# abdur75648/AI-Camera

Hardware: AMD Instinct MI355X
Metric: end-to-end frames/sec @1280x720, 30 persons/frame (higher is better)
Workload: dtype f16

## Files before the change

### ai-camera_amd/csrc/kernels_conv_block.hip

```cpp
#include "conv_common.hpp"

namespace aic {

struct BlockArgs {
    const void* x; void* y;
    const void* w1; const float* b1;
    const void* w2; const float* b2;
    const void* zero;
    int x_cs, x_coff, y_cs, y_coff, H, n_img, ipb;
    const int* n_dev;
};

__global__ __launch_bounds__(512) void conv3x3_c64_block_kernel(const BlockArgs a) {
    constexpr int PW = 34, ROWB = PW * 128, IN_ROWS = 20, MID_ROWS = 16;
    constexpr int MID_OFF = IN_ROWS * ROWB, DUMMY_OFF = MID_OFF + MID_ROWS * ROWB, BIAS_OFF = DUMMY_OFF + 1024;
    extern __shared__ __attribute__((aligned(16))) char smem[];

    const int t = threadIdx.x, lane = t & 63, wv = __builtin_amdgcn_readfirstlane(t >> 6), r = lane & 15, q = lane >> 4;
    const int grp = wv >> 2, cx = wv & 1, ch = (wv >> 1) & 1;
    const half_t* __restrict__ xg = reinterpret_cast<const half_t*>(a.x);
    const half_t* zero = reinterpret_cast<const half_t*>(a.zero);
    const half_t* __restrict__ wg = reinterpret_cast<const half_t*>(grp ? a.w2 : a.w1);
    const float* bg = grp ? a.b2 : a.b1;

    half8 wreg[18][2];
#pragma unroll
    for (int j = 0; j < 2; ++j) {
        const half_t* wr = wg + (size_t)(32 * ch + perm_row<2>(j, r)) * 576 + 8 * q;
#pragma unroll
        for (int s2 = 0; s2 < 18; ++s2) wreg[s2][j] = *reinterpret_cast<const half8*>(wr + 32 * s2);
    }
#pragma unroll
    for (int s2 = 0; s2 < 18; ++s2) asm volatile("" :: "v"(wreg[s2][0]), "v"(wreg[s2][1]));
    float* bias_l = reinterpret_cast<float*>(smem + BIAS_OFF) + ((grp * 2 + ch) * 4 + q) * 8;
    if (cx == 0 && r == 0) {
#pragma unroll
        for (int j = 0; j < 2; ++j)
#pragma unroll
            for (int e = 0; e < 4; ++e) bias_l[4 * j + e] = bg[32 * ch + perm_ch<2>(j, q, e)];
    }
    for (int o = t * 16; o < MID_ROWS * ROWB; o += 512 * 16) *reinterpret_cast<uint4*>(smem + MID_OFF + o) = make_uint4(0u, 0u, 0u, 0u);

    const int gpi = a.H / 4 + 1;
    const int n_live = a.n_dev ? min(a.n_img, a.n_dev[0]) : a.n_img;
    const int ipb = a.n_dev ? (n_live + (int)gridDim.x - 1) / (int)gridDim.x : a.ipb;
    const int img0 = blockIdx.x * ipb;
    const int n_loc = max(0, min(ipb, n_live - img0));
    const int S_tot = gpi * n_loc;

    int doff[3];
#pragma unroll
    for (int p = 0; p < 3; ++p) {
        const int sl = (p * 8 + wv) * 64 + lane;
        const int rr = sl / 272, rem = sl - rr * 272;
        const int px = rem >> 3, c = (rem & 7) ^ (px & 7);
        doff[p] = (p * 8 + wv < 17 && (unsigned)(px - 1) < 32u) ? (rr * 32 + (px - 1)) * a.x_cs + a.x_coff + c * 8 : -1;
    }
    auto issue = [&](int g) {
        int gs = g % 5; if (gs < 0) gs += 5;
        const int jl = g >= 0 ? g / gpi : 0, gy = g - jl * gpi;
        const bool real = g >= 0 && jl < n_loc && gy < gpi - 1;
        const half_t* gbase = xg + ((size_t)(img0 + jl) * a.H + gy * 4) * 32 * a.x_cs;
#pragma unroll
        for (int p = 0; p < 3; ++p) {
            const int j = p * 8 + wv;
            const half_t* src = (real && doff[p] >= 0) ? gbase + doff[p] : zero;
            asm volatile("" : "+v"(src));
            char* dst = j < 17 ? smem + gs * 4 * ROWB + j * 1024 : smem + DUMMY_OFF;
            __builtin_amdgcn_global_load_lds((gptr_t)src, (lptr_t)dst, 16, 0, 0);
        }
    };

    int xk[3];
#pragma unroll
    for (int kw = 0; kw < 3; ++kw) {
        const int px = cx * 16 + r + kw;
        xk[kw] = (px * 8 + (q ^ (px & 7))) * 16;
    }
    const int px1 = cx * 16 + r + 1;
    const int mid_w = (px1 * 8 + ((4 * ch + q) ^ (px1 & 7))) * 16;

    half_t* yg = reinterpret_cast<half_t*>(a.y);
    const unsigned yl0 = (unsigned)((((cx * 16 + r) * a.y_cs) + a.y_coff + 32 * ch + 8 * q) * 2);
    const unsigned rl0 = (unsigned)((((cx * 16 + r) * a.x_cs) + a.x_coff + 32 * ch + 8 * q) * 2);
    const unsigned ystep = (unsigned)(32 * a.y_cs * 2), rstep = (unsigned)(32 * a.x_cs * 2);

    floatx4 acc[4][2];
    half8 rv[4];
    half8 xf[6];
    int rowb[6];
    auto xread = [&xf, &xk, &rowb](auto g, auto ir) {
        constexpr int gg = decltype(g)::value, ii = decltype(ir)::value, kw = gg >> 1;
        const int ad = ((gg & 1) ? (xk[kw] ^ 64) : xk[kw]) + rowb[ii];
        asm volatile("ds_read_b128 %0, %1" : "=v"(xf[ii]) : "v"(ad));
    };
    auto xwait = [&xf](auto n, auto ir) {
        asm volatile("s_waitcnt lgkmcnt(%1)" : "+v"(xf[decltype(ir)::value]) : "n"(decltype(n)::value));
    };
    auto kfirst = [&]() {
        static_for<6>([&](auto ir) { xread(std::integral_constant<int, 0>{}, ir); });
#pragma unroll
        for (int i = 0; i < 4; ++i)
#pragma unroll
            for (int j = 0; j < 2; ++j) acc[i][j] = *reinterpret_cast<const floatx4*>(bias_l + 4 * j);
    };
    auto kpart = [&](auto part) {
        static_for<3>([&](auto gi) {
            constexpr int g = 3 * decltype(part)::value + decltype(gi)::value, kw = g >> 1, cc = g & 1;
            static_for<6>([&](auto ir_c) {
                constexpr int ir = decltype(ir_c)::value;
                xwait(std::integral_constant<int, (g == 5 ? 5 - ir : 5)>{}, ir_c);
#pragma unroll
                for (int kh = 0; kh < 3; ++kh) {
                    const int i = ir - kh;
                    if (i < 0 || i > 3) continue;
#pragma unroll
                    for (int j = 0; j < 2; ++j)
                        acc[i][j] = __builtin_amdgcn_mfma_f32_16x16x32_f16(wreg[(kh * 3 + kw) * 2 + cc][j], xf[ir], acc[i][j], 0, 0, 0);
                }
                if constexpr (g + 1 < 6) xread(std::integral_constant<int, g + 1>{}, ir_c);
                __builtin_amdgcn_sched_barrier(0);
            });
        });
    };
    using P0 = std::integral_constant<int, 0>;
    using P1 = std::integral_constant<int, 1>;

    auto rows1 = [&](int s) {
#pragma unroll
        for (int ir = 0; ir < 6; ++ir) {
            const int v = 4 * s - 1 + ir;
            int gsl = (v >> 2) % 5; if (gsl < 0) gsl += 5;
            rowb[ir] = (gsl * 4 + (v & 3)) * ROWB;
        }
    };
    auto store_mid = [&](int s) {
#pragma unroll
        for (int i = 0; i < 4; ++i) {
            float v[8];
#pragma unroll
            for (int e = 0; e < 8; ++e) v[e] = act_fast<2>(acc[i][e >> 2][e & 3]);
            const half8 o = {(half_t)v[0], (half_t)v[1], (half_t)v[2], (half_t)v[3], (half_t)v[4], (half_t)v[5], (half_t)v[6], (half_t)v[7]};
            const int ad = MID_OFF + ((4 * s + i) & 15) * ROWB + mid_w;
            asm volatile("ds_write_b128 %0, %1" :: "v"(ad), "v"(o) : "memory");
        }
    };
    auto zero_mid = [&](int s) {
        const half8 o = {0, 0, 0, 0, 0, 0, 0, 0};
#pragma unroll
        for (int i = 0; i < 4; ++i) {
            const int ad = MID_OFF + ((4 * s + i) & 15) * ROWB + mid_w;
            asm volatile("ds_write_b128 %0, %1" :: "v"(ad), "v"(o) : "memory");
        }
    };
    auto load_res = [&](size_t pix0) {
        const char* rb = reinterpret_cast<const char*>(xg) + pix0 * a.x_cs * 2;
        unsigned rl = rl0;
        asm volatile("" : "+v"(rl));
#pragma unroll
        for (int i = 0; i < 4; ++i)
            asm volatile("global_load_dwordx4 %0, %1, %2" : "=v"(rv[i]) : "v"(rl + i * rstep), "s"(rb) : "memory");
    };
    auto rows2 = [&](int tt) {
#pragma unroll
        for (int ir = 0; ir < 6; ++ir) rowb[ir] = MID_OFF + ((4 * tt - 1 + ir) & 15) * ROWB;
    };
    auto store_out = [&](size_t pix0) {
        asm volatile("s_waitcnt vmcnt(3)" : "+v"(rv[0]), "+v"(rv[1]), "+v"(rv[2]), "+v"(rv[3]) :: "memory");
        char* yb = reinterpret_cast<char*>(yg) + pix0 * a.y_cs * 2;
        unsigned yl = yl0;
        asm volatile("" : "+v"(yl));
#pragma unroll
        for (int i = 0; i < 4; ++i) {
            float v[8];
#pragma unroll
            for (int e = 0; e < 8; ++e) v[e] = act_fast<2>(acc[i][e >> 2][e & 3] + (float)rv[i][e]);
            const half8 o = {(half_t)v[0], (half_t)v[1], (half_t)v[2], (half_t)v[3], (half_t)v[4], (half_t)v[5], (half_t)v[6], (half_t)v[7]};
            *reinterpret_cast<half8*>(yb + (size_t)(yl + i * ystep)) = o;
        }
    };

    issue(-1); issue(0); issue(1); issue(2);
    asm volatile("s_waitcnt lgkmcnt(0)" ::: "memory");
    if (grp == 0) {
        for (int s = 0; s < S_tot + 2; ++s) {
            wait_vmcnt<3>();
            __builtin_amdgcn_s_barrier();
            issue(s + 3);
            const bool live = s < S_tot, act1 = live && s % gpi < gpi - 1;
            if (act1) {
                rows1(s);
                kfirst();
                kpart(P0{});
            }
            __builtin_amdgcn_s_barrier();
            if (live) {
                if (act1) {
                    kpart(P1{});
                    store_mid(s);
                } else zero_mid(s);
                asm volatile("s_waitcnt lgkmcnt(0)" ::: "memory");
            }
        }
        __builtin_amdgcn_s_barrier();
    } else {
        wait_vmcnt<3>();
        __builtin_amdgcn_s_barrier();
        bool prev = false;
        for (int s = 0; s < S_tot + 2; ++s) {
            __builtin_amdgcn_s_barrier();
            const int tt = s - 2;
            const bool act2 = tt >= 0 && tt < S_tot && (tt % gpi) < gpi - 1;
            const int jl = act2 ? tt / gpi : 0, gy = act2 ? tt % gpi : 0;
            const size_t pix0 = ((size_t)(img0 + jl) * a.H + gy * 4) * 32;
            if (act2) load_res(pix0);
            issue(s + 3);
            if (act2) {
                rows2(tt);
                kfirst();
                kpart(P0{});
            }
            if (act2 && prev) wait_vmcnt<11>();
            else if (act2 || prev) wait_vmcnt<7>();
            else wait_vmcnt<3>();
            __builtin_amdgcn_s_barrier();
            if (act2) {
                kpart(P1{});
                store_out(pix0);
            }
            prev = act2;
        }
    }
    wait_vmcnt<0>();
}

void launch_c64_block(const ConvArgs& c1, const ConvArgs& c2, int ipb, hipStream_t s) {
    BlockArgs a{};
    a.x = c1.x, a.y = c2.y, a.w1 = c1.w, a.b1 = c1.bias, a.w2 = c2.w, a.b2 = c2.bias, a.zero = c1.zero;
    a.x_cs = c1.x_cs, a.x_coff = c1.x_coff, a.y_cs = c2.y_cs, a.y_coff = c2.y_coff, a.H = c1.H;
    a.n_img = c1.M / (c1.H * c1.W);
    a.n_dev = c1.n_dev;
    a.ipb = ipb;
    constexpr size_t lds = (size_t)(20 + 16) * 34 * 128 + 1024 + 512;
    set_lds_limit(conv3x3_c64_block_kernel, lds);
    hipLaunchKernelGGL(conv3x3_c64_block_kernel, dim3((a.n_img + a.ipb - 1) / a.ipb), dim3(512), lds, s, a);
    KCHECK();
}

}
```

Before: 13120.

## Interleave epilogue stores with final MFMA group and strength-reduce block conv indexing

The fused two-conv block kernel now emits the mid-row LDS writes and output global stores inside the last MFMA group instead of after it, so the epilogue overlaps with matrix work. Bias initialisation is done through two LDS reads feeding the first MFMA accumulator. Per-step divisions and modulos for slot and row addressing are replaced with incrementally updated counters and pointers. Wave priority is raised around the second half. Optional compile-time timestamp instrumentation is added but disabled by default. The waitcnt arithmetic gets more intricate, which raises the risk of ordering mistakes.

```diff
diff --git a/ai-camera_amd/csrc/kernels_conv_block.hip b/ai-camera_amd/csrc/kernels_conv_block.hip
--- a/ai-camera_amd/csrc/kernels_conv_block.hip
+++ b/ai-camera_amd/csrc/kernels_conv_block.hip
@@ -1,6 +1,25 @@
 #include "conv_common.hpp"
 
 namespace aic {
+
+#ifdef AICAM_BLOCK_STAMPS
+constexpr int STAMP_BLOCKS = 1536, STAMP_WORDS = 16;
+__device__ unsigned long long aic_block_stamp_buf[STAMP_BLOCKS * 8 * STAMP_WORDS];
+struct BlockStamps { unsigned long long t[6], sum[6], steps, last, t_begin, rt_begin; bool have; };
+#define BLK_STAMP(k) do { __builtin_amdgcn_sched_barrier(0); asm volatile("s_memtime %0\n\ts_waitcnt lgkmcnt(0)" : "=s"(st.t[k]) :: "memory"); __builtin_amdgcn_sched_barrier(0); } while (0)
+#define BLK_TOP() do { if (st.have) st.sum[5] += st.t[0] - st.last; st.have = false; } while (0)
+#define BLK_STEP() do { for (int k_ = 0; k_ < 5; ++k_) st.sum[k_] += st.t[k_ + 1] - st.t[k_]; ++st.steps; st.last = st.t[5]; st.have = true; } while (0)
+#define BLK_STAMPS_BEGIN() BlockStamps st{}; asm volatile("s_memtime %0\n\ts_memrealtime %1\n\ts_waitcnt lgkmcnt(0)" : "=s"(st.t_begin), "=s"(st.rt_begin) :: "memory")
+#define BLK_STAMPS_OUT() do { unsigned long long te_, re_; asm volatile("s_memtime %0\n\ts_memrealtime %1\n\ts_waitcnt lgkmcnt(0)" : "=s"(te_), "=s"(re_) :: "memory"); \
+        if (lane == 0 && blockIdx.x < STAMP_BLOCKS) { unsigned long long* o_ = aic_block_stamp_buf + ((size_t)blockIdx.x * 8 + wv) * STAMP_WORDS; \
+            for (int k_ = 0; k_ < 6; ++k_) o_[k_] = st.sum[k_]; o_[6] = st.steps; o_[7] = te_ - st.t_begin; o_[8] = re_ - st.rt_begin; } } while (0)
+#else
+#define BLK_STAMP(k) do {} while (0)
+#define BLK_TOP() do {} while (0)
+#define BLK_STEP() do {} while (0)
+#define BLK_STAMPS_BEGIN() do {} while (0)
+#define BLK_STAMPS_OUT() do {} while (0)
+#endif
 
 struct BlockArgs {
     const void* x; void* y;
@@ -39,6 +58,7 @@
 #pragma unroll
             for (int e = 0; e < 4; ++e) bias_l[4 * j + e] = bg[32 * ch + perm_ch<2>(j, q, e)];
     }
+    const int bias_ad = BIAS_OFF + ((grp * 2 + ch) * 4 + q) * 32;
     for (int o = t * 16; o < MID_ROWS * ROWB; o += 512 * 16) *reinterpret_cast<uint4*>(smem + MID_OFF + o) = make_uint4(0u, 0u, 0u, 0u);
 
     const int gpi = a.H / 4 + 1;
@@ -56,11 +76,7 @@
         const int px = rem >> 3, c = (rem & 7) ^ (px & 7);
         doff[p] = (p * 8 + wv < 17 && (unsigned)(px - 1) < 32u) ? (rr * 32 + (px - 1)) * a.x_cs + a.x_coff + c * 8 : -1;
     }
-    auto issue = [&](int g) {
-        int gs = g % 5; if (gs < 0) gs += 5;
-        const int jl = g >= 0 ? g / gpi : 0, gy = g - jl * gpi;
-        const bool real = g >= 0 && jl < n_loc && gy < gpi - 1;
-        const half_t* gbase = xg + ((size_t)(img0 + jl) * a.H + gy * 4) * 32 * a.x_cs;
+    auto issue_at = [&](int gs, bool real, const half_t* gbase) {
 #pragma unroll
         for (int p = 0; p < 3; ++p) {
             const int j = p * 8 + wv;
@@ -70,6 +86,16 @@
             __builtin_amdgcn_global_load_lds((gptr_t)src, (lptr_t)dst, 16, 0, 0);
         }
     };
+    int i_gs = 4, i_jl = 0, i_gy = -1;
+    const half_t* i_ptr = xg + (size_t)img0 * a.H * 32 * a.x_cs;
+    const size_t i_step = (size_t)4 * 32 * a.x_cs;
+    auto issue_next = [&]() {
+        const bool real = i_gy >= 0 && i_jl < n_loc && i_gy < gpi - 1;
+        issue_at(i_gs, real, i_ptr);
+        if (i_gy >= 0 && i_gy < gpi - 1) i_ptr += i_step;
+        i_gs = i_gs == 4 ? 0 : i_gs + 1;
+        if (++i_gy == gpi) i_gy = 0, ++i_jl;
+    };
 
     int xk[3];
 #pragma unroll
@@ -89,6 +115,7 @@
     half8 rv[4];
     half8 xf[6];
     int rowb[6];
+    BLK_STAMPS_BEGIN();
     auto xread = [&xf, &xk, &rowb](auto g, auto ir) {
         constexpr int gg = decltype(g)::value, ii = decltype(ir)::value, kw = gg >> 1;
         const int ad = ((gg & 1) ? (xk[kw] ^ 64) : xk[kw]) + rowb[ii];
@@ -98,52 +125,55 @@
         asm volatile("s_waitcnt lgkmcnt(%1)" : "+v"(xf[decltype(ir)::value]) : "n"(decltype(n)::value));
     };
     auto kfirst = [&]() {
+        asm volatile("ds_read_b128 %0, %1" : "=v"(acc[3][0]) : "v"(bias_ad));
+        asm volatile("ds_read_b128 %0, %1 offset:16" : "=v"(acc[3][1]) : "v"(bias_ad));
         static_for<6>([&](auto ir) { xread(std::integral_constant<int, 0>{}, ir); });
-#pragma unroll
-        for (int i = 0; i < 4; ++i)
-#pragma unroll
-            for (int j = 0; j < 2; ++j) acc[i][j] = *reinterpret_cast<const floatx4*>(bias_l + 4 * j);
-    };
-    auto kpart = [&](auto part) {
+    };
+    auto kpart = [&](auto part, auto lds_writes, auto&& tail) {
         static_for<3>([&](auto gi) {
             constexpr int g = 3 * decltype(part)::value + decltype(gi)::value, kw = g >> 1, cc = g & 1;
             static_for<6>([&](auto ir_c) {
                 constexpr int ir = decltype(ir_c)::value;
-                xwait(std::integral_constant<int, (g == 5 ? 5 - ir : 5)>{}, ir_c);
+                constexpr int wr = g == 5 && decltype(lds_writes)::value && ir > 2 ? ir - 2 : 0;
+                xwait(std::integral_constant<int, (g == 5 ? 5 - ir + wr : 5)>{}, ir_c);
+                if constexpr (g == 0 && ir == 0) asm volatile("" : "+v"(acc[3][0]), "+v"(acc[3][1]));
 #pragma unroll
                 for (int kh = 0; kh < 3; ++kh) {
                     const int i = ir - kh;
                     if (i < 0 || i > 3) continue;
 #pragma unroll
                     for (int j = 0; j < 2; ++j)
-                        acc[i][j] = __builtin_amdgcn_mfma_f32_16x16x32_f16(wreg[(kh * 3 + kw) * 2 + cc][j], xf[ir], acc[i][j], 0, 0, 0);
+                        acc[i][j] = __builtin_amdgcn_mfma_f32_16x16x32_f16(wreg[(kh * 3 + kw) * 2 + cc][j], xf[ir], (g == 0 && kh == 0) ? acc[3][j] : acc[i][j], 0, 0, 0);
                 }
                 if constexpr (g + 1 < 6) xread(std::integral_constant<int, g + 1>{}, ir_c);
                 __builtin_amdgcn_sched_barrier(0);
+                if constexpr (g == 5 && ir == 5) BLK_STAMP(4);
+                if constexpr (g == 5 && ir >= 2) {
+                    tail(std::integral_constant<int, ir - 2>{});
+                    __builtin_amdgcn_sched_barrier(0);
+                }
             });
         });
     };
     using P0 = std::integral_constant<int, 0>;
     using P1 = std::integral_constant<int, 1>;
-
-    auto rows1 = [&](int s) {
-#pragma unroll
-        for (int ir = 0; ir < 6; ++ir) {
-            const int v = 4 * s - 1 + ir;
-            int gsl = (v >> 2) % 5; if (gsl < 0) gsl += 5;
-            rowb[ir] = (gsl * 4 + (v & 3)) * ROWB;
-        }
-    };
-    auto store_mid = [&](int s) {
-#pragma unroll
-        for (int i = 0; i < 4; ++i) {
-            float v[8];
-#pragma unroll
-            for (int e = 0; e < 8; ++e) v[e] = act_fast<2>(acc[i][e >> 2][e & 3]);
-            const half8 o = {(half_t)v[0], (half_t)v[1], (half_t)v[2], (half_t)v[3], (half_t)v[4], (half_t)v[5], (half_t)v[6], (half_t)v[7]};
-            const int ad = MID_OFF + ((4 * s + i) & 15) * ROWB + mid_w;
-            asm volatile("ds_write_b128 %0, %1" :: "v"(ad), "v"(o) : "memory");
-        }
+    auto no_tail = [](auto) {};
+
+    auto rows1 = [&](int s5) {
+        const int up = s5 == 0 ? 4 : s5 - 1, dn = s5 == 4 ? 0 : s5 + 1;
+        rowb[0] = (up * 4 + 3) * ROWB;
+#pragma unroll
+        for (int ir = 1; ir < 5; ++ir) rowb[ir] = (s5 * 4 + ir - 1) * ROWB;
+        rowb[5] = dn * 4 * ROWB;
+    };
+    auto mid_row = [&](int s, auto ic) {
+        constexpr int i = decltype(ic)::value;
+        float v[8];
+#pragma unroll
+        for (int e = 0; e < 8; ++e) v[e] = act_fast<2>(acc[i][e >> 2][e & 3]);
+        const half8 o = {(half_t)v[0], (half_t)v[1], (half_t)v[2], (half_t)v[3], (half_t)v[4], (half_t)v[5], (half_t)v[6], (half_t)v[7]};
+        const int ad = MID_OFF + ((4 * s + i) & 15) * ROWB + mid_w;
+        asm volatile("ds_write_b128 %0, %1" :: "v"(ad), "v"(o) : "memory");
     };
     auto zero_mid = [&](int s) {
         const half8 o = {0, 0, 0, 0, 0, 0, 0, 0};
@@ -153,8 +183,7 @@
             asm volatile("ds_write_b128 %0, %1" :: "v"(ad), "v"(o) : "memory");
         }
     };
-    auto load_res = [&](size_t pix0) {
-        const char* rb = reinterpret_cast<const char*>(xg) + pix0 * a.x_cs * 2;
+    auto load_res = [&](const char* rb) {
         unsigned rl = rl0;
         asm volatile("" : "+v"(rl));
 #pragma unroll
@@ -165,73 +194,92 @@
 #pragma unroll
         for (int ir = 0; ir < 6; ++ir) rowb[ir] = MID_OFF + ((4 * tt - 1 + ir) & 15) * ROWB;
     };
-    auto store_out = [&](size_t pix0) {
-        asm volatile("s_waitcnt vmcnt(3)" : "+v"(rv[0]), "+v"(rv[1]), "+v"(rv[2]), "+v"(rv[3]) :: "memory");
-        char* yb = reinterpret_cast<char*>(yg) + pix0 * a.y_cs * 2;
+    auto out_row = [&](char* yb, auto ic) {
+        constexpr int i = decltype(ic)::value;
+        if constexpr (i == 0) asm volatile("s_waitcnt vmcnt(3)" : "+v"(rv[0]), "+v"(rv[1]), "+v"(rv[2]), "+v"(rv[3]) :: "memory");
         unsigned yl = yl0;
         asm volatile("" : "+v"(yl));
-#pragma unroll
-        for (int i = 0; i < 4; ++i) {
-            float v[8];
-#pragma unroll
-            for (int e = 0; e < 8; ++e) v[e] = act_fast<2>(acc[i][e >> 2][e & 3] + (float)rv[i][e]);
-            const half8 o = {(half_t)v[0], (half_t)v[1], (half_t)v[2], (half_t)v[3], (half_t)v[4], (half_t)v[5], (half_t)v[6], (half_t)v[7]};
-            *reinterpret_cast<half8*>(yb + (size_t)(yl + i * ystep)) = o;
-        }
-    };
-
-    issue(-1); issue(0); issue(1); issue(2);
+        float v[8];
+#pragma unroll
+        for (int e = 0; e < 8; ++e) v[e] = act_fast<2>(acc[i][e >> 2][e & 3] + (float)rv[i][e]);
+        const half8 o = {(half_t)v[0], (half_t)v[1], (half_t)v[2], (half_t)v[3], (half_t)v[4], (half_t)v[5], (half_t)v[6], (half_t)v[7]};
+        *reinterpret_cast<half8*>(yb + (size_t)(yl + i * ystep)) = o;
+    };
+
+    issue_next(); issue_next(); issue_next(); issue_next();
     asm volatile("s_waitcnt lgkmcnt(0)" ::: "memory");
     if (grp == 0) {
+        int sy = 0, s5 = 0;
         for (int s = 0; s < S_tot + 2; ++s) {
             wait_vmcnt<3>();
             __builtin_amdgcn_s_barrier();
-            issue(s + 3);
-            const bool live = s < S_tot, act1 = live && s % gpi < gpi - 1;
+            BLK_STAMP(0);
+            BLK_TOP();
+            issue_next();
+            const bool live = s < S_tot, act1 = live && sy < gpi - 1;
             if (act1) {
-                rows1(s);
+                BLK_STAMP(1);
+                rows1(s5);
                 kfirst();
-                kpart(P0{});
+                kpart(P0{}, std::true_type{}, no_tail);
+                BLK_STAMP(2);
             }
             __builtin_amdgcn_s_barrier();
             if (live) {
                 if (act1) {
-                    kpart(P1{});
-                    store_mid(s);
+                    BLK_STAMP(3);
+                    __builtin_amdgcn_s_setprio(1);
+                    kpart(P1{}, std::true_type{}, [&](auto i) { mid_row(s, i); });
+                    __builtin_amdgcn_s_setprio(0);
                 } else zero_mid(s);
                 asm volatile("s_waitcnt lgkmcnt(0)" ::: "memory");
+                if (act1) { BLK_STAMP(5); BLK_STEP(); }
             }
+            sy = sy + 1 == gpi ? 0 : sy + 1;
+            s5 = s5 == 4 ? 0 : s5 + 1;
         }
         __builtin_amdgcn_s_barrier();
     } else {
         wait_vmcnt<3>();
         __builtin_amdgcn_s_barrier();
         bool prev = false;
+        int ty = 0;
+        const char* rb = reinterpret_cast<const char*>(xg) + (size_t)img0 * a.H * 32 * a.x_cs * 2;
+        char* yb = reinterpret_cast<char*>(yg) + (size_t)img0 * a.H * 32 * a.y_cs * 2;
         for (int s = 0; s < S_tot + 2; ++s) {
             __builtin_amdgcn_s_barrier();
+            BLK_STAMP(0);
+            BLK_TOP();
             const int tt = s - 2;
-            const bool act2 = tt >= 0 && tt < S_tot && (tt % gpi) < gpi - 1;
-            const int jl = act2 ? tt / gpi : 0, gy = act2 ? tt % gpi : 0;
-            const size_t pix0 = ((size_t)(img0 + jl) * a.H + gy * 4) * 32;
-            if (act2) load_res(pix0);
-            issue(s + 3);
+            const bool act2 = tt >= 0 && tt < S_tot && ty < gpi - 1;
+            if (act2) load_res(rb);
+            issue_next();
             if (act2) {
+                BLK_STAMP(1);
                 rows2(tt);
                 kfirst();
-                kpart(P0{});
+                kpart(P0{}, std::false_type{}, no_tail);
+                BLK_STAMP(2);
             }
             if (act2 && prev) wait_vmcnt<11>();
             else if (act2 || prev) wait_vmcnt<7>();
             else wait_vmcnt<3>();
             __builtin_amdgcn_s_barrier();
             if (act2) {
-                kpart(P1{});
-                store_out(pix0);
+                BLK_STAMP(3);
+                __builtin_amdgcn_s_setprio(1);
+                kpart(P1{}, std::false_type{}, [&](auto i) { out_row(yb, i); });
+                __builtin_amdgcn_s_setprio(0);
+                BLK_STAMP(5);
+                BLK_STEP();
+                rb += (size_t)4 * rstep, yb += (size_t)4 * ystep;
             }
             prev = act2;
+            if (tt >= 0) ty = ty + 1 == gpi ? 0 : ty + 1;
         }
     }
     wait_vmcnt<0>();
+    BLK_STAMPS_OUT();
 }
 
 void launch_c64_block(const ConvArgs& c1, const ConvArgs& c2, int ipb, hipStream_t s) {
@@ -248,3 +296,9 @@
 }
 
 }
+
+#ifdef AICAM_BLOCK_STAMPS
+extern "C" int aic_block_stamps_read(unsigned long long* out, long words) {
+    return (int)hipMemcpyFromSymbol(out, HIP_SYMBOL(aic::aic_block_stamp_buf), (size_t)words * sizeof(unsigned long long));
+}
+#endif
```

Measured after the change: 13250 (median of 6 runs). About the same (+1.0%).
